# tdavchev/DESIRE

Measured on AMD Instinct MI355X. Metric: agent-trajectory-samples/sec (K=20, T_pred=40), higher is better.
Workload: dtype f32; 1 GPU; BASELINE configs[1]: SDD-like synthetic windows, 32 agent slots/window, K=20, T_obs=8/T_pred=40, H=128, L=128, fp32, posterior CVAE, IOC 1 refinement, social grid 4x4, scene grid 64x64x32; 512 windows/step/GPU; windows_per_gpu=512, rows_per_gpu=327680, parallelism=scene-sharded x1

## Files before the change

### desire_amd/csrc/api_forward.hip

```cpp
#include "ctx.h"

#include <cmath>
#include <cstdio>
#include <cstdlib>
#include <cstring>

bool compact_rows(const desire_ctx* h) { return (h->d.flags & DESIRE_FLAG_COMPACT_ROWS) != 0; }
bool compact_ioc(const desire_ctx* h) { return (h->d.flags & DESIRE_FLAG_COMPACT_IOC) && ioc_plan(h).fwd != IocFwd::STEPWISE; }
ClassLayout class_layout(const desire_ctx* h, bool pad, const int* counts) {
    const desire_dims& d = h->d;
    ClassLayout L;
    int cand[6], nc = 0;
    for (int m : {8, 10, 16, 32, 64, 96}) if (m < d.mno && (m != 10 || pad)) cand[nc++] = m;
    for (int i = nc > 3 ? nc - 3 : 0; i < nc; ++i) L.m[L.n++] = cand[i];
    L.m[L.n++] = d.mno;
    for (int i = L.n; i < 4; ++i) L.m[i] = d.mno;
    for (int c = 0; c < L.n; ++c) {
        IocView& v = L.c[c];
        v.cls = c; v.mno = L.m[c]; v.n_scenes = counts ? counts[c] : d.n_scenes;
        v.gpt = (v.mno <= 32 && 32 % v.mno) ? 32 / v.mno : 0; v.ngrp = v.n_scenes * d.K;
        v.R = v.gpt ? (long)((v.ngrp + v.gpt - 1) / v.gpt) * 32 : (long)v.ngrp * v.mno;
        v.agent_off = L.agents; v.row_off = L.rows; v.win_off = L.wins;
        L.agents += (size_t)v.n_scenes * v.mno; L.rows += (size_t)v.R; L.wins += (size_t)v.n_scenes;
    }
// ... 302 lines not shown

int ioc_cluster_exchange(desire_ctx* h, size_t n_groups, bool reset_err, hipStream_t s) {
    if (!h->ws.count("hex") && (h->ws["hex"].alloc((size_t)2 * h->R * h->d.H * sizeof(float)) || h->ws["grp_cnt"].alloc(((size_t)h->R / 32 + 1) * sizeof(int)) ||
                                h->ws["ioc_err"].alloc(sizeof(int))))
        return fail(DESIRE_ERR_HIP, "hipMalloc failed for the cluster exchange buffers");
    HIPCHK(hipMemsetAsync(h->ws["grp_cnt"].p, 0, n_groups * sizeof(int), s));
    if (reset_err) HIPCHK(hipMemsetAsync(h->ws["ioc_err"].p, 0, sizeof(int), s));
    return DESIRE_OK;
}
int ioc_cluster_check(desire_ctx* h, hipStream_t s, const char* what) {
    int err = 0;
    HIPCHK(hipMemcpyAsync(&err, h->ws["ioc_err"].p, sizeof(int), hipMemcpyDeviceToHost, s));
    HIPCHK(hipStreamSynchronize(s));
    return err ? fail(DESIRE_ERR_HIP, std::string(what) + " hand-off timed out (workgroups of a group were not co-resident)") : DESIRE_OK;
}
#ifdef DESIRE_IOC_TIMING
void ioc_timing_report(const long long* dbg, const char* const* names, int n, hipStream_t s) {
    long long host[16];
    (void)hipStreamSynchronize(s); (void)hipMemcpy(host, dbg, n * sizeof(long long), hipMemcpyDeviceToHost);
    long long tot = 0; for (int k = 0; k < n; ++k) tot += host[k];
    for (int k = 0; k < n; ++k) fprintf(stderr, "[ioc timing] %-45s %12lld cyc  %5.1f%%\n", names[k], host[k], 100.0 * host[k] / (double)tot);
}
#endif

static int ioc_core(desire_handle* h, const IocView& v, hipStream_t s) {
    const desire_dims& d = h->d;
    if (h->training && d.bf16 == 1) return fail(DESIRE_ERR_STATE, "bf16 operands are inference-only");
    IocArgs a{};
    a.Y = v.Y; a.score = v.score; a.Hx = v.Hx; a.ldhx = 2 * d.H; a.p_last = v.p_last; a.valid = v.valid;
    a.R = (int)v.R; a.K = d.K; a.mno = v.mno; a.H = d.H; a.T = d.T_pred; a.iters = d.iters;
    a.C = d.C; a.Gh = d.Gh; a.Gw = d.Gw; a.E_v = d.E_v; a.G = d.grid_size; a.nb_w = d.nb_w; a.nb_h = d.nb_h;
    a.grids = h->grids; a.grid_of_scene = v.gos; a.bin_tab = d.bin_mode == 1 ? W(h, "bin_tab") : nullptr;
    a.w_vel = D(h, "ioc/vel_w"); a.b_vel = D(h, "ioc/vel_b");
    a.Wsoc = D4(h, "ioc/Wsoc"); a.b_soc = D(h, "ioc/soc_b"); a.Wsoc_c = D4(h, "ioc/Wsoc_c");
    a.Wg = D4(h, "ioc/Wg"); a.Wc = D4(h, "ioc/Wc"); a.b_g = D(h, "ioc/gb"); a.b_c = D(h, "ioc/cb");
    a.w_score = D(h, "ioc/score_w"); a.b_score = D(h, "ioc/score_b");
    a.Wreg = D4(h, "ioc/Wreg"); a.b_reg = D(h, "ioc/reg_b"); a.NTreg = (2 * d.T_pred + 31) / 32;
    a.variant = d.ioc_form; a.gpt = v.gpt; a.ngrp = v.ngrp; a.dyn = DynCount{v.dynN, 1, 0};
    const IocPlan p = ioc_plan(d, h->training, v.mno, v.gpt, v.R, [&](int n) { return ioc_bin_split_capacity(a, n); });
    if (!p.fp32_weights()) { a.Wsoc = D4(h, "ioc/Wsoc16"); a.Wg = D4(h, "ioc/Wg16"); a.Wc = D4(h, "ioc/Wc16"); a.Wreg = D4(h, "ioc/Wreg16"); }
    if (p.cluster()) {
        if (int rc = ioc_cluster_exchange(h, (size_t)v.R / v.mno, true, s)) return rc;
        a.hex = W(h, "hex"); a.grp_cnt = static_cast<int*>(h->ws["grp_cnt"].p); a.err = static_cast<int*>(h->ws["ioc_err"].p);
    }
    if (p.nspl > 1) {
        const size_t tiles = ((size_t)v.R + 31) / 32, tiles_max = ((size_t)h->R + 31) / 32;
        if ((!h->ws.count("hex_s") || !h->ws["hex_s"].p || !h->ws["cnt_s"].p) &&
            (h->ws["hex_s"].alloc(tiles_max * 2 * 4 * 32 * d.H * sizeof(float)) || h->ws["cnt_s"].alloc(tiles_max * sizeof(int))))
            return fail(DESIRE_ERR_HIP, "hipMalloc failed for the bin-split exchange buffers");
        if (!h->host_err) {
            if (hipHostMalloc(reinterpret_cast<void**>(&h->host_err), sizeof(int), hipHostMallocMapped) != hipSuccess || !h->host_err)
                { h->host_err = nullptr; return fail(DESIRE_ERR_HIP, "hipHostMalloc failed for the bin-split error word"); }
            *h->host_err = 0;
        }
        if (*static_cast<volatile int*>(h->host_err)) {
            *h->host_err = 0;
            return fail(DESIRE_ERR_HIP, "bin-split IOC hand-off timed out in an earlier call (workgroups of a tile were not co-resident)");
        }
        launch_fill_f32(W(h, "cnt_s"), tiles, 0.f, s);
        a.hex = W(h, "hex_s"); a.grp_cnt = static_cast<int*>(h->ws["cnt_s"].p); a.err = h->host_err;
        a.nspl = p.nspl;
    }
#ifdef DESIRE_IOC_TIMING
    if (!h->ws.count("dbg")) { h->ws["dbg"].alloc(10 * sizeof(long long)); }
    a.dbg = static_cast<long long*>(h->ws["dbg"].p);
#endif
    const int passes = h->training ? d.iters : 1;
// ... 130 lines not shown
```

### desire_amd/csrc/api_pack.hip

```cpp
#include "ctx.h"

#include <cmath>
#include <cstdio>
#include <cstdlib>
#include <cstring>

namespace {
void fold_bn(desire_ctx* h, const std::string& p, std::vector<float>& scale, std::vector<float>& shift) {
    const auto& g = h->host_w.at(p + "/bn/gamma"); const auto& be = h->host_w.at(p + "/bn/beta");
    const auto& mu = h->host_w.at(p + "/bn/moving_mean"); const auto& var = h->host_w.at(p + "/bn/moving_var");
    const auto& b = h->host_w.at(p + "/b");
    scale.resize(g.size()); shift.resize(g.size());
    for (size_t i = 0; i < g.size(); ++i) {
        const double sc = (double)g[i] / std::sqrt((double)var[i] + 1e-3);
        scale[i] = (float)sc;
        shift[i] = (float)((double)be[i] + sc * ((double)b[i] - (double)mu[i]));
    }
}

}

int desire_pack_all(desire_ctx* h) {
    const desire_dims& d = h->d;
    const int H = d.H, L = d.L, V = h->V, E = h->E, B = h->B;
// ... 200 lines not shown
                return out;
            };
            bad |= up("vae_enc/conv2/W16", fwd16(hw["vae_enc/conv2/w"], 32, 64));
            bad |= up("vae_enc/conv3/W16", fwd16(hw["vae_enc/conv3/w"], 64, 128));
        }
        bad |= up("vae_dec/deconv2/W16", taps16(hw["vae_dec/deconv2/w"], 128, 64));
        bad |= up("vae_dec/deconv3/W16", taps16(hw["vae_dec/deconv3/w"], 64, 32));
        {
            const auto& w4 = hw["vae_dec/deconv4/w"];
            bad |= up("vae_dec/deconv4/W16", pack_b16(32, 32, chain, [&](int k, int n) { return n < 25 ? w4[(size_t)n * 32 + k] : 0.f; }));
        }
    }
    bad |= up("ioc/vel_w", hw["ioc/vel_fc/w"]); bad |= up("ioc/vel_b", hw["ioc/vel_fc/b"]);
    {
        std::vector<float> all;
        for (int b = 0; b < B; ++b) {
            auto pk = pack_b(H, H, rowmajor(hw["ioc/social_fc/w"], H, b * H));
            all.insert(all.end(), pk.begin(), pk.end());
        }
        bad |= up("ioc/Wsoc", all);
    }
    {
        const auto& ws = hw["ioc/social_fc/w"];
        const int T16 = H / 16;
        std::vector<float> all((size_t)B * H * H);
        for (int b = 0; b < B; ++b)
            for (int ct = 0; ct < T16; ++ct)
                for (int g = 0; g < T16; ++g)
                    for (int lane = 0; lane < 64; ++lane)
                        for (int j = 0; j < 4; ++j)
                            all[((((size_t)b * T16 + ct) * T16 + g) * 64 + lane) * 4 + j] =
                                ws[((size_t)b * H + 16 * g + 4 * (lane >> 4) + j) * H + 16 * ct + (lane & 15)];
        bad |= up("ioc/Wsoc_c", all);
    }
    bad |= up("ioc/soc_b", hw["ioc/social_fc/b"]);
    bad |= up("ioc/score_w", hw["ioc/score/w"]); bad |= up("ioc/score_b", hw["ioc/score/b"]);
    bad |= up("ioc/Wreg", pack_b(H, 2 * d.T_pred, rowmajor(hw["ioc/reg/w"], 2 * d.T_pred, 0)));
    bad |= up("ioc/reg_b", hw["ioc/reg/b"]);
    bad |= up("fc_c/W", pack_b(2 * H, V, rowmajor(hw["fc_c/w"], V, 0)));  bad |= up("fc_c/b", hw["fc_c/b"]);
    bad |= up("vae_enc/fc/W", pack_b(2048, 2 * L, rowmajor(hw["vae_enc/fc/w"], 2 * L, 0)));
    bad |= up("vae_enc/fc/b", hw["vae_enc/fc/b"]);
    bad |= up("mask/W", pack_b(V, H, rowmajor(hw["mask_fc/w"], H, 0)));  bad |= up("mask/b", hw["mask_fc/b"]);
    std::vector<float> sc, sh;
    for (const char* n : {"vae_enc/conv1", "vae_enc/conv2", "vae_enc/conv3", "vae_dec/deconv1", "vae_dec/deconv2",
                          "vae_dec/deconv3", "vae_dec/deconv4"}) {
        fold_bn(h, n, sc, sh);
        bad |= up(std::string(n) + "/scale", sc); bad |= up(std::string(n) + "/shift", sh);
        if (d.bn_mode != 0) { bad |= up(std::string(n) + "/gamma", hw[std::string(n) + "/bn/gamma"]); bad |= up(std::string(n) + "/beta", hw[std::string(n) + "/bn/beta"]); }
    }
    bad |= up("vae_enc/conv1/raw", hw["vae_enc/conv1/w"]);
    bad |= up("vae_dec/deconv4/raw", hw["vae_dec/deconv4/w"]);
    auto pack_taps = [&](const std::vector<float>& w, int CI, int CO, bool transposed) {
        std::vector<float> all;
        for (int tap = 0; tap < 25; ++tap) {
            const float* base = w.data() + (size_t)tap * CI * CO;
            auto pk = pack_b(CI, CO, [&](int k, int n) { return transposed ? base[(size_t)n * CI + k] : base[(size_t)k * CO + n]; });
            all.insert(all.end(), pk.begin(), pk.end());
        }
        return all;
    };
    bad |= up("vae_enc/conv2/W", pack_taps(hw["vae_enc/conv2/w"], 32, 64, false));
    bad |= up("vae_enc/conv3/W", pack_taps(hw["vae_enc/conv3/w"], 64, 128, false));
    bad |= up("vae_dec/deconv2/W", pack_taps(hw["vae_dec/deconv2/w"], 128, 64, true));
    bad |= up("vae_dec/deconv3/W", pack_taps(hw["vae_dec/deconv3/w"], 64, 32, true));
    {
        const auto& w1 = hw["vae_dec/deconv1/w"];
// ... 22 lines not shown
```

### desire_amd/csrc/kernels.h

```cpp
#pragma once
#include <hip/hip_runtime.h>
#include <stdint.h>

template <class F>
inline void allow_big_lds(F* f) {
    static bool done = false;
    if (!done) {
        (void)hipFuncSetAttribute(reinterpret_cast<const void*>(f), hipFuncAttributeMaxDynamicSharedMemorySize, 160 * 1024);
        done = true;
    }
}

struct DynCount { const int32_t* cnt; int mul; int hint; };
inline int dyn_units(int worst, const DynCount& d) {
    if (!d.cnt || d.hint <= 0) return worst;
    const long g = (long)d.hint * d.mul, want = g + g / 4 + 256;
    return (int)(want < (long)worst ? want : (long)worst);
}

enum { EPI_BIAS = 0, EPI_BIAS_RELU = 1, EPI_SCALE_SHIFT_ELU = 2, EPI_NONE = 3, EPI_ELUGRAD = 4, EPI_SIGGRAD = 5 };

struct GemmArgs {
    const float* A; int lda; int M; int K;
    const float4* Bp; int G; int NT;
// ... 47 lines not shown
    uint8_t* valid;
    float* sv_r; float* sv_u; float* sv_c; float* sv_h; float* sv_x;
    int n_roll; const float* w5; const float* b5;
    const float* normals; float* roll_out;
    DynCount dyn;
};
void launch_encoder(const EncArgs& a, hipStream_t s);
void launch_encoder_pair(const EncArgs& past, const EncArgs& fut, hipStream_t s);
void launch_encoder_bf16(const EncArgs& a, hipStream_t s);

struct DecArgs {
    const float* xz; const float* Hx; int ldhx; const float* p_last;
    int R; int K; int mno; int H; int T;
    const float4* Wxg; const float4* Wxc; const float4* Whg; const float4* Whc;
    const float* b_g; const float* b_c;
    const float* w_head; const float* b_head;
    float* Y;
    float* hdump;
    float* sv_r; float* sv_u; float* sv_c;
    DynCount dyn;
};
void launch_decoder(const DecArgs& a, hipStream_t s);
void launch_decoder_bf16(const DecArgs& a, hipStream_t s);

struct IocArgs {
    float* Y; float* score;
    const float* Hx; int ldhx; const float* p_last; const uint8_t* valid;
    int R; int K; int mno; int H; int T; int iters;
    int C; int Gh; int Gw; int E_v; int G; float nb_w, nb_h;
    const float* grids; const int32_t* grid_of_scene;
    const float* w_vel; const float* b_vel;
    const float4* Wsoc; const float* b_soc;
    const float4* Wsoc_c;
    const float4* Wg; const float4* Wc; const float* b_g; const float* b_c;
    const float* w_score; const float* b_score;
    const float4* Wreg; const float* b_reg; int NTreg;
    int variant;
    long long* dbg;
    float* hex; int* grp_cnt; int* err;
    int nspl;
    float* sv_x; float* sv_r; float* sv_u; float* sv_c; float* sv_h;
    const float* bin_tab;
    int gpt; int ngrp;
    DynCount dyn;
};
void launch_ioc(const IocArgs& a, bool wide, hipStream_t s);
void launch_ioc_cluster(const IocArgs& a, hipStream_t s);
int ioc_bin_split_capacity(const IocArgs& a, int n);
void launch_ioc_bf16(const IocArgs& a, bool wide, hipStream_t s);
int launch_ioc_bf16_cluster(const IocArgs& a, hipStream_t s);
void launch_ioc_x3(const IocArgs& a, hipStream_t s);
void launch_ioc_x6(const IocArgs& a, hipStream_t s);
void launch_ioc_x6r2(const IocArgs& a, hipStream_t s);
void launch_ioc_x3r2(const IocArgs& a, hipStream_t s);
bool decoder_x6_supported(int H);
void launch_decoder_x6(const DecArgs& a, hipStream_t s, int np = 3);
void launch_deconv2_x6(const ConvArgs& a, hipStream_t s, int np = 3);
void launch_deconv3_x6(const ConvArgs& a, hipStream_t s, int np = 3);
struct IocStepArgs {
    int t; int rank; int nranks; int m_loc; int n_scenes; int K; int R;
    int H; int T; int Gh; int Gw; int G; float nb_w, nb_h;
    const float* Yall; const float* plast_all; const uint8_t* valid_all; const float* Hall;
    int peer; const float* Yp[8]; const float* plp[8]; const uint8_t* vp[8]; const float* Hp[8];
    const float* st_h; float* st_h_out; float* st_score; float* st_h_copy;
    const float* grids; const int32_t* grid_of_scene;
    const float* w_vel; const float* b_vel; const float4* Wsoc; const float* b_soc;
// ... 138 lines not shown
```

### desire_amd/csrc/kernels_rnn.hip

```cpp
#include "common.h"
#include "kernels.h"
#include <cstdlib>
#include <map>
#include <tuple>

#define RNN_WG 512

__device__ __forceinline__ f32x16 splat16(float v) {
    f32x16 z;
#pragma unroll
    for (int i = 0; i < 16; ++i) z[i] = v;
    return z;
}

__device__ __forceinline__ void mma1(f32x16& acc, const float* a_lane, const float4* __restrict__ b_lane, int G) {
    f32x16 t[1] = {acc};
    mma_groups<1>(t, a_lane, 0, b_lane, G);
    acc = t[0];
}

template <int H, int TM, bool ROLL>
__device__ __forceinline__ void encoder_tile(const EncArgs& a, int blk) {
    extern __shared__ __attribute__((aligned(16))) float smem[];
    constexpr int LDH = H + 4, NT = H >> 5, G = H >> 3, NTHR = NT * (TM / 32) * 64;
// ... 289 lines not shown
    }
}
template <int H, int TM>
static void launch_decoder_t(const DecArgs& a, hipStream_t s) {
    const size_t lds = (2 * TM * (H + 4) + 2 * H + TM * 2) * sizeof(float);
    if (a.sv_r || a.sv_c || a.hdump) {
        allow_big_lds(k_decoder<H, TM, true>);
        hipLaunchKernelGGL((k_decoder<H, TM, true>), dim3((a.R + TM - 1) / TM), dim3((H / 32) * (TM / 32) * 64), lds, s, a);
    } else {
        allow_big_lds(k_decoder<H, TM, false>);
        hipLaunchKernelGGL((k_decoder<H, TM, false>), dim3((a.R + TM - 1) / TM), dim3((H / 32) * (TM / 32) * 64), lds, s, a);
    }
}
void launch_decoder(const DecArgs& a, hipStream_t s) {
    if (a.H == 256) launch_decoder_t<256, 32>(a, s);
    else if (a.H == 128) {
        launch_decoder_t<128, 32>(a, s);
    }
    else launch_decoder_t<64, 64>(a, s);
}

#include "cluster.h"
#include "split.h"
template <int TM> struct MaskT { typedef unsigned long long type; };
template <> struct MaskT<32> { typedef unsigned type; };
__device__ __forceinline__ int ffs_(unsigned m) { return __ffs((int)m); }
__device__ __forceinline__ int ffs_(unsigned long long m) { return __ffsll((long long)m); }
#ifdef DESIRE_IOC_TIMING
#define TICK(k) { const long long now_ = clock64(); tacc[k] += now_ - tprev; tprev = now_; }
#else
#define TICK(k)
#endif
typedef float f32x4v __attribute__((ext_vector_type(4)));
template <int H, int EV, int C, int TM, bool TRAIN, bool CP = false, int NSPL = 1, bool PAD = false>
__global__ __launch_bounds__((H / 32) * (TM / 32) * 64, ((H / 32) * (TM / 32) <= 2) ? 1 : 2) void k_ioc(IocArgs a) {
#ifdef DESIRE_IOC_TIMING
    long long tacc[10] = {0, 0, 0, 0, 0, 0, 0, 0, 0, 0};
    long long tprev = clock64();
#endif
    extern __shared__ __attribute__((aligned(16))) float smem[];
    constexpr int NT = H >> 5, E = EV + C + H, KX = E + H, LDX = KX + 4, LDB = H + 4;
    constexpr int NTHR = NT * (TM / 32) * 64, TPR = NTHR / TM;
    constexpr int G8 = KX >> 3, GH = H >> 3;
    constexpr int NCH = H / (4 * TPR);
    const int B = a.G * a.G;
    float* XH = smem;
    float* AB = XH + (TM + 1) * LDX;
    typedef typename MaskT<TM>::type mask_t;
    mask_t* masks = reinterpret_cast<mask_t*>(AB + 2 * TM * LDB);
    float* pc = reinterpret_cast<float*>(masks + TM * B);
    float* pp = pc + TM * 2;
    float* wv = pp + TM * 2;
    float* red = wv + 3 * EV;
    unsigned char* vld = reinterpret_cast<unsigned char*>(red + NT * TM);
    unsigned* occ = reinterpret_cast<unsigned*>(vld + TM);
    unsigned* rowbits = occ + 2;
    unsigned* rowlist = rowbits + 36;

    const int lane = lane_id(), w = wave_id(), tid = threadIdx.x;
    const int cb = w % NT, mt = w / NT;
    const int tile = NSPL > 1 ? (int)blockIdx.x / NSPL : (int)blockIdx.x, member = NSPL > 1 ? (int)blockIdx.x % NSPL : 0;
    const int row0 = tile * TM;
    IOC_DYN(a)
    if (a.dyn.cnt && row0 >= a.R) return;
    unsigned long long my_bins = ~0ull;
    if (NSPL > 1) { my_bins = 0ull; for (int b = member; b < 64; b += NSPL) my_bins |= 1ull << b; }
    const bool active = cb < NT;
    const int col = cb * 32 + (lane & 31);
// ... 23 lines not shown
    constexpr int NS = 2;
    auto build = [&](int b, int buf) {
        float* ab = AB + buf * TM * LDB + r8 * LDB;
        mask_t m2 = masks[r8 * B + b];
        int off[NS];
#pragma unroll
        for (int sl = 0; sl < NS; ++sl) {
            off[sl] = m2 ? (grp_base + ffs_(m2) - 1) * LDX : TM * LDX;
            m2 &= m2 - 1;
        }
        float4 s[NCH];
#pragma unroll
        for (int c = 0; c < NCH; ++c) {
            const float4 v0 = *reinterpret_cast<const float4*>(XH + off[0] + E + q8 * 4 + c * 4 * TPR);
            const float4 v1 = *reinterpret_cast<const float4*>(XH + off[1] + E + q8 * 4 + c * 4 * TPR);
            s[c].x = v0.x + v1.x; s[c].y = v0.y + v1.y; s[c].z = v0.z + v1.z; s[c].w = v0.w + v1.w;
        }
        if (__any(m2 != 0)) {
            while (m2) {
                const int j = ffs_(m2) - 1;
                m2 &= m2 - 1;
                const float* src = XH + (grp_base + j) * LDX + E + q8 * 4;
#pragma unroll
                for (int c = 0; c < NCH; ++c) {
                    const float4 v = *reinterpret_cast<const float4*>(src + c * 4 * TPR);
                    s[c].x += v.x; s[c].y += v.y; s[c].z += v.z; s[c].w += v.w;
                }
            }
        }
#pragma unroll
        for (int c = 0; c < NCH; ++c) *reinterpret_cast<float4*>(ab + q8 * 4 + c * 4 * TPR) = s[c];
    };

    for (int it = 0; it < a.iters; ++it) {
        for (int i = tid; i < TM * (H >> 2); i += NTHR) {
            const int r = i / (H >> 2), c4 = i - r * (H >> 2);
            const int ag = ioc_agent_of_row(min(row0 + r, a.R - 1), a.K, a.mno, gpt, a.ngrp);
            *reinterpret_cast<float4*>(XH + r * LDX + E + c4 * 4) =
                ag >= 0 ? *reinterpret_cast<const float4*>(a.Hx + (size_t)ag * a.ldhx + c4 * 4) : make_float4(0.f, 0.f, 0.f, 0.f);
        }
        if (tid < TM) {
            const int ag = ioc_agent_of_row(min(row0 + tid, a.R - 1), a.K, a.mno, gpt, a.ngrp);
            pp[tid * 2] = ag >= 0 ? a.p_last[(size_t)ag * 2] : 0.f;
            pp[tid * 2 + 1] = ag >= 0 ? a.p_last[(size_t)ag * 2 + 1] : 0.f;
        }
        __syncthreads();
        f32x16 h = zero16(), sp = zero16();
        if (active) {
#pragma unroll
            for (int i = 0; i < 16; ++i) h[i] = my_x[((i & 3) + 8 * (i >> 2)) * LDX + E];
        }

        float2 ynext = make_float2(0.f, 0.f);
        if (tid < TM) {
            const float2 y0 = *reinterpret_cast<const float2*>(a.Y + ((size_t)min(row0 + tid, a.R - 1) * a.T) * 2);
            pc[tid * 2] = y0.x; pc[tid * 2 + 1] = y0.y;
        }
        for (int i = tid; i < TM * B; i += NTHR) masks[i] = 0;
        if (tid < 2) occ[tid] = 0;
        if (CP && tid < B) rowbits[tid] = 0;
        __syncthreads();
        const float* rh_lane = AB + (mt * 32 + (lane & 31)) * LDB + 4 * (lane >> 5);
        float* my_rh = AB + (mt * 32 + 4 * (lane >> 5)) * LDB + col;
        constexpr int GX = E >> 3;

        for (int t = 0; t < a.T; ++t) {
            TICK(0)
            if (tid < TM && t + 1 < a.T)
                ynext = *reinterpret_cast<const float2*>(a.Y + ((size_t)min(row0 + tid, a.R - 1) * a.T + t + 1) * 2);
            {
                const float px = pc[r8 * 2], py = pc[r8 * 2 + 1];
                const float vx = px - pp[r8 * 2], vy = py - pp[r8 * 2 + 1];
                constexpr int per = EV / TPR;
#pragma unroll
                for (int j = q8 * per; j < (q8 + 1) * per; ++j)
                    XH[r8 * LDX + j] = fmaxf(fmaf(vy, wv[EV + j], vx * wv[j]) + wv[2 * EV + j], 0.f);
                int cy, cx;
                scene_cell_dev(px, py, a.Gh, a.Gw, cy, cx);
                const float* gsrc = grid + ((size_t)cy * a.Gw + cx) * C;
                constexpr int cper = C / TPR;
                if (cper >= 4) {
#pragma unroll
                    for (int j = q8 * cper; j < (q8 + 1) * cper; j += 4)
                        *reinterpret_cast<float4*>(XH + r8 * LDX + EV + j) = *reinterpret_cast<const float4*>(gsrc + j);
                } else {
                    *reinterpret_cast<float2*>(XH + r8 * LDX + EV + q8 * 2) = *reinterpret_cast<const float2*>(gsrc + q8 * 2);
                }
                float nbw, nbh;
                nb_opaque(a.nb_w, a.nb_h, nbw, nbh);
                const unsigned long long oc = nb_search<4>(pc, vld, grp_base, n_nb, q8, TPR, my_slot, px, py, nbw, nbh, a.G, a.bin_tab,
                                                          [&](int j, int b) {
                                                              atomicOr(&masks[r8 * B + b], (mask_t)1 << j);
                                                              if (CP) atomicOr(&rowbits[b], 1u << r8);
                                                          });
                nb_publish_occ(oc, occ, B);
                if (CP) {
#pragma unroll
                    for (int c = 0; c < NCH; ++c)
                        *reinterpret_cast<float4*>(XH + r8 * LDX + EV + C + q8 * 4 + c * 4 * TPR) = make_float4(0.f, 0.f, 0.f, 0.f);
                }
            }
            __syncthreads();
            TICK(1)
            if constexpr (CP) {
                unsigned long long om = (unsigned long long)__builtin_amdgcn_readfirstlane((int)occ[0]) & 0xffffffffull;
                om |= (unsigned long long)(unsigned)__builtin_amdgcn_readfirstlane((int)occ[1]) << 32;
                constexpr int T16 = H / 16;
                auto build_c = [&](int b, int buf) {
                    const unsigned rb = rowbits[b];
                    if (!((rb >> r8) & 1u)) return;
                    const int slot = __popc(rb & ((1u << r8) - 1u));
                    float* ab = AB + buf * TM * LDB + slot * LDB;
                    mask_t m2 = masks[r8 * B + b];
                    const int o0 = (grp_base + ffs_(m2) - 1) * LDX;
                    m2 &= m2 - 1;
                    const int o1 = m2 ? (grp_base + ffs_(m2) - 1) * LDX : TM * LDX;
                    m2 &= m2 - 1;
                    float4 sacc[NCH];
#pragma unroll
                    for (int c = 0; c < NCH; ++c) {
                        const float4 v0 = *reinterpret_cast<const float4*>(XH + o0 + E + q8 * 4 + c * 4 * TPR);
                        const float4 v1 = *reinterpret_cast<const float4*>(XH + o1 + E + q8 * 4 + c * 4 * TPR);
                        sacc[c].x = v0.x + v1.x; sacc[c].y = v0.y + v1.y; sacc[c].z = v0.z + v1.z; sacc[c].w = v0.w + v1.w;
                    }
                    while (m2) {
                        const int j = ffs_(m2) - 1;
                        m2 &= m2 - 1;
                        const float* src = XH + (grp_base + j) * LDX + E + q8 * 4;
#pragma unroll
                        for (int c = 0; c < NCH; ++c) {
                            const float4 v = *reinterpret_cast<const float4*>(src + c * 4 * TPR);
                            sacc[c].x += v.x; sacc[c].y += v.y; sacc[c].z += v.z; sacc[c].w += v.w;
                        }
                    }
#pragma unroll
                    for (int c = 0; c < NCH; ++c) *reinterpret_cast<float4*>(ab + q8 * 4 + c * 4 * TPR) = sacc[c];
                    if (q8 == 0) reinterpret_cast<unsigned char*>(rowlist + buf * (TM / 4))[slot] = (unsigned char)r8;
                };
                int buf = 0;
                if (om) build_c(ffs_(om) - 1, 0);
                __syncthreads();
                while (om) {
                    const int b = ffs_(om) - 1;
                    om &= om - 1;
                    const float4* w0 = a.Wsoc_c + ((size_t)(b * T16 + 2 * cb) * T16) * 64 + lane;
                    float4 wf[2][T16];
                    if (active) {
#pragma unroll
                        for (int g = 0; g < T16; ++g) { wf[0][g] = w0[g * 64]; wf[1][g] = w0[(T16 + g) * 64]; }
                    }
                    if (om) build_c(ffs_(om) - 1, buf ^ 1);
                    const int nrows = __popc(__builtin_amdgcn_readfirstlane((int)rowbits[b]));
                    if (active) {
                        for (int c16 = 0; c16 * 16 < nrows; ++c16) {
                            f32x4v a0 = {0.f, 0.f, 0.f, 0.f}, a1 = {0.f, 0.f, 0.f, 0.f};
                            const float* ap = AB + buf * TM * LDB + (16 * c16 + (lane & 15)) * LDB + 4 * (lane >> 4);
#pragma unroll
                            for (int g = 0; g < T16; ++g) {
                                const float4 av = *reinterpret_cast<const float4*>(ap + 16 * g);
                                a0 = __builtin_amdgcn_mfma_f32_16x16x4f32(av.x, wf[0][g].x, a0, 0, 0, 0);
                                a1 = __builtin_amdgcn_mfma_f32_16x16x4f32(av.x, wf[1][g].x, a1, 0, 0, 0);
                                a0 = __builtin_amdgcn_mfma_f32_16x16x4f32(av.y, wf[0][g].y, a0, 0, 0, 0);
                                a1 = __builtin_amdgcn_mfma_f32_16x16x4f32(av.y, wf[1][g].y, a1, 0, 0, 0);
                                a0 = __builtin_amdgcn_mfma_f32_16x16x4f32(av.z, wf[0][g].z, a0, 0, 0, 0);
                                a1 = __builtin_amdgcn_mfma_f32_16x16x4f32(av.z, wf[1][g].z, a1, 0, 0, 0);
                                a0 = __builtin_amdgcn_mfma_f32_16x16x4f32(av.w, wf[0][g].w, a0, 0, 0, 0);
                                a1 = __builtin_amdgcn_mfma_f32_16x16x4f32(av.w, wf[1][g].w, a1, 0, 0, 0);
                            }
                            const unsigned rl4 = rowlist[buf * (TM / 4) + 4 * c16 + (lane >> 4)];
                            float* ex = XH + EV + C + cb * 32 + (lane & 15);
#pragma unroll
// ... 101 lines not shown
                }
#pragma unroll
                for (int i = 0; i < 16; ++i) my_rh[((i & 3) + 8 * (i >> 2)) * LDB] = rh[i];
#pragma unroll
                for (int i = 0; i < 16; ++i) {
                    u[i] = sigmoidf_(u[i] + bgu);
                    if (TRAIN && row0 + mt * 32 + acc_row(i) < a.R) sv_u_t[sv_off(i, t)] = u[i];
                }
            }
            __syncthreads();
            TICK(7)
            if (active) {
                f32x16 ac = zero16();
                mma1(ac, x_lane, a.Wc + ((size_t)cb * G8) * 64 + lane, GX);
                mma1(ac, rh_lane, a.Wc + ((size_t)cb * G8 + GX) * 64 + lane, GH);
#pragma unroll
                for (int i = 0; i < 16; ++i) {
                    const float c = tanhf_(ac[i] + bcc);
                    h[i] = gru_blend(u[i], h[i], c);
                    sp[i] = fmaf(h[i], wsc, sp[i]);
                    if (TRAIN && row0 + mt * 32 + acc_row(i) < a.R) { sv_c_t[sv_off(i, t)] = c; sv_h_t[sv_off(i, t)] = h[i]; }
                }
#pragma unroll
                for (int i = 0; i < 16; ++i)
                    my_x[((i & 3) + 8 * (i >> 2)) * LDX + E] = h[i];
            }
            __builtin_amdgcn_s_setprio(0);
            if (tid < TM) {
                pp[tid * 2] = pc[tid * 2]; pp[tid * 2 + 1] = pc[tid * 2 + 1];
                pc[tid * 2] = ynext.x; pc[tid * 2 + 1] = ynext.y;
            }
            for (int i = tid; i < TM * B; i += NTHR) masks[i] = 0;
            if (tid < 2) occ[tid] = 0;
            if (CP && tid < B) rowbits[tid] = 0;
            __syncthreads();
            TICK(8)
        }
#pragma unroll
        for (int i = 0; i < 16; ++i) {
            float v = active ? sp[i] : 0.f;
            v += __shfl_xor(v, 1); v += __shfl_xor(v, 2); v += __shfl_xor(v, 4);
            v += __shfl_xor(v, 8); v += __shfl_xor(v, 16);
            if ((lane & 31) == 0) red[cb * TM + mt * 32 + acc_row(i)] = v;
        }
        __syncthreads();
        bool poisoned = false;
        if constexpr (NSPL > 1) poisoned = __hip_atomic_load(a.err, __ATOMIC_RELAXED, __HIP_MEMORY_SCOPE_SYSTEM) != 0;
        if (tid < TM && row0 + tid < a.R && it == a.iters - 1 && member == 0) {
            float sc = 0.f;
#pragma unroll
            for (int c = 0; c < NT; ++c) sc += red[c * TM + tid];
            a.score[row0 + tid] = poisoned ? __builtin_nanf("") : sc + (float)a.T * a.b_score[0];
        }
        for (int nt = cb; nt < a.NTreg; nt += NT) {
            f32x16 acc = zero16();
            mma1(acc, x_lane + E, a.Wreg + ((size_t)nt * GH) * 64 + lane, GH);
            const int cc = nt * 32 + (lane & 31);
            if (cc < 2 * a.T) {
                const float bb = a.b_reg[cc];
#pragma unroll
                for (int i = 0; i < 16; ++i) {
                    const int row = row0 + mt * 32 + acc_row(i);
                    if (row < a.R && member == 0) {
                        float* y = a.Y + (size_t)row * 2 * a.T + cc;
                        *y = poisoned ? __builtin_nanf("") : *y + (acc[i] + bb);
                    }
                }
// ... 26 lines not shown
            if (a.variant != 9) {
                allow_big_lds(k_ioc<H, 16, 32, 32, true, true>);
                hipLaunchKernelGGL((k_ioc<H, 16, 32, 32, true, true>), grid, block, ioc_lds_bytes(a, TM), s, a);
                return;
            }
        }
        if constexpr (H <= 128 || TM == 32) {
            allow_big_lds(k_ioc<H, 16, 32, TM, true>);
            hipLaunchKernelGGL((k_ioc<H, 16, 32, TM, true>), grid, block, ioc_lds_bytes(a, TM), s, a);
        }
        return;
    }
    if constexpr (TM == 32 && H <= 128) {
        if (a.variant == 8) {
            allow_big_lds(k_ioc<H, 16, 32, 32, false, true>);
            hipLaunchKernelGGL((k_ioc<H, 16, 32, 32, false, true>), grid, block, ioc_lds_bytes(a, TM), s, a);
            return;
        }
    }
    if constexpr (TM == 32 && H <= 128) {
        if (a.nspl > 1) {
            const dim3 gs(grid.x * a.nspl);
            switch (a.nspl) {
                case 3: allow_big_lds(k_ioc<H, 16, 32, 32, false, false, 3>); hipLaunchKernelGGL((k_ioc<H, 16, 32, 32, false, false, 3>), gs, block, ioc_lds_bytes(a, TM), s, a); return;
                case 4: allow_big_lds(k_ioc<H, 16, 32, 32, false, false, 4>); hipLaunchKernelGGL((k_ioc<H, 16, 32, 32, false, false, 4>), gs, block, ioc_lds_bytes(a, TM), s, a); return;
                default: allow_big_lds(k_ioc<H, 16, 32, 32, false, false, 2>); hipLaunchKernelGGL((k_ioc<H, 16, 32, 32, false, false, 2>), gs, block, ioc_lds_bytes(a, TM), s, a); return;
            }
        }
    }
    if constexpr (TM == 32 && H <= 128) {
        if (a.gpt > 0) {
            allow_big_lds(k_ioc<H, 16, 32, 32, false, false, 1, true>);
            hipLaunchKernelGGL((k_ioc<H, 16, 32, 32, false, false, 1, true>), grid, block, ioc_lds_bytes(a, TM), s, a);
            return;
        }
    }
    allow_big_lds(k_ioc<H, 16, 32, TM, false>);
    hipLaunchKernelGGL((k_ioc<H, 16, 32, TM, false>), grid, block, ioc_lds_bytes(a, TM), s, a);
}
int ioc_bin_split_capacity(const IocArgs& a, int n) {
    if (a.mno > 32 || a.H > 128 || n < 2 || n > 4) return 0;
    static std::map<std::tuple<int, int, int, size_t>, int> cache;
    int dev = 0;
    if (hipGetDevice(&dev) != hipSuccess) return 0;
    const size_t lds = ioc_lds_bytes(a, 32);
    const auto key = std::make_tuple(dev, a.H, n, lds);
    auto it = cache.find(key);
    if (it != cache.end()) return it->second;
    const void* kern = nullptr;
    if (a.H == 128) kern = n == 2 ? (const void*)k_ioc<128, 16, 32, 32, false, false, 2> : n == 3 ? (const void*)k_ioc<128, 16, 32, 32, false, false, 3> : (const void*)k_ioc<128, 16, 32, 32, false, false, 4>;
    else kern = n == 2 ? (const void*)k_ioc<64, 16, 32, 32, false, false, 2> : n == 3 ? (const void*)k_ioc<64, 16, 32, 32, false, false, 3> : (const void*)k_ioc<64, 16, 32, 32, false, false, 4>;
    (void)hipFuncSetAttribute(kern, hipFuncAttributeMaxDynamicSharedMemorySize, 160 * 1024);
    int per_cu = 0, cus = 0;
    int cap = 0;
    if (hipOccupancyMaxActiveBlocksPerMultiprocessor(&per_cu, kern, (a.H / 32) * 64, lds) == hipSuccess && per_cu > 0 &&
        hipDeviceGetAttribute(&cus, hipDeviceAttributeMultiprocessorCount, dev) == hipSuccess)
        cap = per_cu * cus;
    cache[key] = cap;
    return cap;
}
void launch_ioc(const IocArgs& a, bool wide, hipStream_t s) {
    if (a.H == 256) launch_ioc_t<256, 32>(a, s);
    else if (a.H == 128) { if (wide) launch_ioc_t<128, 64>(a, s); else launch_ioc_t<128, 32>(a, s); }
    else { if (wide) launch_ioc_t<64, 64>(a, s); else launch_ioc_t<64, 32>(a, s); }
}

// ... 854 lines not shown
```

Before: 2.417 million samples/s.

## Add row-sparse social pooling path to IOC kernel using compacted per-bin row lists

Adds an SP template variant of the IOC kernel that pools only the rows that actually have neighbours in each occupied bin. Those rows are gathered into compacted 16-row MFMA tiles, instead of running the full 32-row tile for every occupied bin. A new Wsoc_s weight layout with a permuted k ordering is packed to match this gather scheme. The build_c lambda is hoisted so it can be shared with the existing compact path. The new path is dispatched for non-padded inference when the variant is not 9. The aim is to cut wasted MFMA work on sparse neighbour bins, at the cost of extra gather/scatter LDS traffic and added synchronisation per bin.

```diff
diff --git a/desire_amd/csrc/api_forward.hip b/desire_amd/csrc/api_forward.hip
--- a/desire_amd/csrc/api_forward.hip
+++ b/desire_amd/csrc/api_forward.hip
@@ -358,7 +358,7 @@
     a.C = d.C; a.Gh = d.Gh; a.Gw = d.Gw; a.E_v = d.E_v; a.G = d.grid_size; a.nb_w = d.nb_w; a.nb_h = d.nb_h;
     a.grids = h->grids; a.grid_of_scene = v.gos; a.bin_tab = d.bin_mode == 1 ? W(h, "bin_tab") : nullptr;
     a.w_vel = D(h, "ioc/vel_w"); a.b_vel = D(h, "ioc/vel_b");
-    a.Wsoc = D4(h, "ioc/Wsoc"); a.b_soc = D(h, "ioc/soc_b"); a.Wsoc_c = D4(h, "ioc/Wsoc_c");
+    a.Wsoc = D4(h, "ioc/Wsoc"); a.b_soc = D(h, "ioc/soc_b"); a.Wsoc_c = D4(h, "ioc/Wsoc_c"); a.Wsoc_s = D4(h, "ioc/Wsoc_s");
     a.Wg = D4(h, "ioc/Wg"); a.Wc = D4(h, "ioc/Wc"); a.b_g = D(h, "ioc/gb"); a.b_c = D(h, "ioc/cb");
     a.w_score = D(h, "ioc/score_w"); a.b_score = D(h, "ioc/score_b");
     a.Wreg = D4(h, "ioc/Wreg"); a.b_reg = D(h, "ioc/reg_b"); a.NTreg = (2 * d.T_pred + 31) / 32;
diff --git a/desire_amd/csrc/api_pack.hip b/desire_amd/csrc/api_pack.hip
--- a/desire_amd/csrc/api_pack.hip
+++ b/desire_amd/csrc/api_pack.hip
@@ -256,6 +256,15 @@
                             all[((((size_t)b * T16 + ct) * T16 + g) * 64 + lane) * 4 + j] =
                                 ws[((size_t)b * H + 16 * g + 4 * (lane >> 4) + j) * H + 16 * ct + (lane & 15)];
         bad |= up("ioc/Wsoc_c", all);
+        for (int b = 0; b < B; ++b)
+            for (int ct = 0; ct < T16; ++ct)
+                for (int g = 0; g < T16; ++g)
+                    for (int lane = 0; lane < 64; ++lane)
+                        for (int j = 0; j < 4; ++j) {
+                            const int q = lane >> 4, k = 16 * g + 8 * (j >> 1) + 2 * (j & 1) + 4 * (q & 1) + (q >> 1);
+                            all[((((size_t)b * T16 + ct) * T16 + g) * 64 + lane) * 4 + j] = ws[((size_t)b * H + k) * H + 16 * ct + (lane & 15)];
+                        }
+        bad |= up("ioc/Wsoc_s", all);
     }
     bad |= up("ioc/soc_b", hw["ioc/social_fc/b"]);
     bad |= up("ioc/score_w", hw["ioc/score/w"]); bad |= up("ioc/score_b", hw["ioc/score/b"]);
diff --git a/desire_amd/csrc/kernels.h b/desire_amd/csrc/kernels.h
--- a/desire_amd/csrc/kernels.h
+++ b/desire_amd/csrc/kernels.h
@@ -103,6 +103,7 @@
     const float* w_vel; const float* b_vel;
     const float4* Wsoc; const float* b_soc;
     const float4* Wsoc_c;
+    const float4* Wsoc_s;
     const float4* Wg; const float4* Wc; const float* b_g; const float* b_c;
     const float* w_score; const float* b_score;
     const float4* Wreg; const float* b_reg; int NTreg;
diff --git a/desire_amd/csrc/kernels_rnn.hip b/desire_amd/csrc/kernels_rnn.hip
--- a/desire_amd/csrc/kernels_rnn.hip
+++ b/desire_amd/csrc/kernels_rnn.hip
@@ -345,8 +345,10 @@
 #define TICK(k)
 #endif
 typedef float f32x4v __attribute__((ext_vector_type(4)));
-template <int H, int EV, int C, int TM, bool TRAIN, bool CP = false, int NSPL = 1, bool PAD = false>
+template <int H, int EV, int C, int TM, bool TRAIN, bool CP = false, int NSPL = 1, bool PAD = false, bool SP = false>
 __global__ __launch_bounds__((H / 32) * (TM / 32) * 64, ((H / 32) * (TM / 32) <= 2) ? 1 : 2) void k_ioc(IocArgs a) {
+    static_assert(!SP || (TM == 32 && !TRAIN && !CP && NSPL == 1), "row-sparse pooling: 32-row inference tiles of the plain form only");
+    constexpr bool RC = CP || SP;
 #ifdef DESIRE_IOC_TIMING
     long long tacc[10] = {0, 0, 0, 0, 0, 0, 0, 0, 0, 0};
     long long tprev = clock64();
@@ -436,6 +438,38 @@
         for (int c = 0; c < NCH; ++c) *reinterpret_cast<float4*>(ab + q8 * 4 + c * 4 * TPR) = s[c];
     };
 
+    auto build_c = [&](int b, int buf) {
+        const unsigned rb = rowbits[b];
+        if (!((rb >> r8) & 1u)) return;
+        const int slot = __popc(rb & ((1u << r8) - 1u));
+        float* ab = AB + buf * TM * LDB + slot * LDB;
+        mask_t m2 = masks[r8 * B + b];
+        const int o0 = (grp_base + ffs_(m2) - 1) * LDX;
+        m2 &= m2 - 1;
+        const int o1 = m2 ? (grp_base + ffs_(m2) - 1) * LDX : TM * LDX;
+        m2 &= m2 - 1;
+        float4 sacc[NCH];
+#pragma unroll
+        for (int c = 0; c < NCH; ++c) {
+            const float4 v0 = *reinterpret_cast<const float4*>(XH + o0 + E + q8 * 4 + c * 4 * TPR);
+            const float4 v1 = *reinterpret_cast<const float4*>(XH + o1 + E + q8 * 4 + c * 4 * TPR);
+            sacc[c].x = v0.x + v1.x; sacc[c].y = v0.y + v1.y; sacc[c].z = v0.z + v1.z; sacc[c].w = v0.w + v1.w;
+        }
+        while (m2) {
+            const int j = ffs_(m2) - 1;
+            m2 &= m2 - 1;
+            const float* src = XH + (grp_base + j) * LDX + E + q8 * 4;
+#pragma unroll
+            for (int c = 0; c < NCH; ++c) {
+                const float4 v = *reinterpret_cast<const float4*>(src + c * 4 * TPR);
+                sacc[c].x += v.x; sacc[c].y += v.y; sacc[c].z += v.z; sacc[c].w += v.w;
+            }
+        }
+#pragma unroll
+        for (int c = 0; c < NCH; ++c) *reinterpret_cast<float4*>(ab + q8 * 4 + c * 4 * TPR) = sacc[c];
+        if (q8 == 0) reinterpret_cast<unsigned char*>(rowlist + buf * (TM / 4))[slot] = (unsigned char)r8;
+    };
+
     for (int it = 0; it < a.iters; ++it) {
         for (int i = tid; i < TM * (H >> 2); i += NTHR) {
             const int r = i / (H >> 2), c4 = i - r * (H >> 2);
@@ -462,7 +496,7 @@
         }
         for (int i = tid; i < TM * B; i += NTHR) masks[i] = 0;
         if (tid < 2) occ[tid] = 0;
-        if (CP && tid < B) rowbits[tid] = 0;
+        if (RC && tid < B) rowbits[tid] = 0;
         __syncthreads();
         const float* rh_lane = AB + (mt * 32 + (lane & 31)) * LDB + 4 * (lane >> 5);
         float* my_rh = AB + (mt * 32 + 4 * (lane >> 5)) * LDB + col;
@@ -495,10 +529,10 @@
                 const unsigned long long oc = nb_search<4>(pc, vld, grp_base, n_nb, q8, TPR, my_slot, px, py, nbw, nbh, a.G, a.bin_tab,
                                                           [&](int j, int b) {
                                                               atomicOr(&masks[r8 * B + b], (mask_t)1 << j);
-                                                              if (CP) atomicOr(&rowbits[b], 1u << r8);
+                                                              if (RC) atomicOr(&rowbits[b], 1u << r8);
                                                           });
                 nb_publish_occ(oc, occ, B);
-                if (CP) {
+                if (RC) {
 #pragma unroll
                     for (int c = 0; c < NCH; ++c)
                         *reinterpret_cast<float4*>(XH + r8 * LDX + EV + C + q8 * 4 + c * 4 * TPR) = make_float4(0.f, 0.f, 0.f, 0.f);
@@ -506,41 +540,77 @@
             }
             __syncthreads();
             TICK(1)
-            if constexpr (CP) {
+            if constexpr (SP) {
                 unsigned long long om = (unsigned long long)__builtin_amdgcn_readfirstlane((int)occ[0]) & 0xffffffffull;
                 om |= (unsigned long long)(unsigned)__builtin_amdgcn_readfirstlane((int)occ[1]) << 32;
                 constexpr int T16 = H / 16;
-                auto build_c = [&](int b, int buf) {
-                    const unsigned rb = rowbits[b];
-                    if (!((rb >> r8) & 1u)) return;
-                    const int slot = __popc(rb & ((1u << r8) - 1u));
-                    float* ab = AB + buf * TM * LDB + slot * LDB;
-                    mask_t m2 = masks[r8 * B + b];
-                    const int o0 = (grp_base + ffs_(m2) - 1) * LDX;
-                    m2 &= m2 - 1;
-                    const int o1 = m2 ? (grp_base + ffs_(m2) - 1) * LDX : TM * LDX;
-                    m2 &= m2 - 1;
-                    float4 sacc[NCH];
-#pragma unroll
-                    for (int c = 0; c < NCH; ++c) {
-                        const float4 v0 = *reinterpret_cast<const float4*>(XH + o0 + E + q8 * 4 + c * 4 * TPR);
-                        const float4 v1 = *reinterpret_cast<const float4*>(XH + o1 + E + q8 * 4 + c * 4 * TPR);
-                        sacc[c].x = v0.x + v1.x; sacc[c].y = v0.y + v1.y; sacc[c].z = v0.z + v1.z; sacc[c].w = v0.w + v1.w;
-                    }
-                    while (m2) {
-                        const int j = ffs_(m2) - 1;
-                        m2 &= m2 - 1;
-                        const float* src = XH + (grp_base + j) * LDX + E + q8 * 4;
-#pragma unroll
-                        for (int c = 0; c < NCH; ++c) {
-                            const float4 v = *reinterpret_cast<const float4*>(src + c * 4 * TPR);
-                            sacc[c].x += v.x; sacc[c].y += v.y; sacc[c].z += v.z; sacc[c].w += v.w;
+                int buf = 0;
+                if (om) build_c(ffs_(om) - 1, 0);
+                __syncthreads();
+                __builtin_amdgcn_s_setprio(3);
+                const int q = lane >> 4;
+                float* ex = XH + EV + C + cb * 32 + (lane & 15);
+                const int kq = 4 * (q & 1) + (q >> 1);
+                float4 wf[2][T16];
+                auto load_w = [&](int b) {
+                    const float4* w0 = a.Wsoc_s + ((size_t)(b * T16 + 2 * cb) * T16) * 64 + lane;
+#pragma unroll
+                    for (int g = 0; g < T16; ++g) { wf[0][g] = w0[g * 64]; wf[1][g] = w0[(T16 + g) * 64]; }
+                };
+                int ro[4];
+                f32x4v a0, a1;
+                auto gather = [&](int c16, int nrows) {
+                    const unsigned rl4 = rowlist[buf * (TM / 4) + 4 * c16 + q];
+#pragma unroll
+                    for (int i = 0; i < 4; ++i) {
+                        ro[i] = 16 * c16 + 4 * q + i < nrows ? (int)((rl4 >> (8 * i)) & 0xffu) * LDX : -1;
+                        a0[i] = ro[i] >= 0 ? ex[ro[i]] : 0.f;
+                        a1[i] = ro[i] >= 0 ? ex[ro[i] + 16] : 0.f;
+                    }
+                };
+                while (om) {
+                    const int b = ffs_(om) - 1;
+                    om &= om - 1;
+                    if (active) load_w(b);
+                    const int nrows = __popc(__builtin_amdgcn_readfirstlane((int)rowbits[b]));
+                    if (om) build_c(ffs_(om) - 1, buf ^ 1);
+                    if (active) {
+                        for (int c16 = 0; c16 * 16 < nrows; ++c16) {
+                            gather(c16, nrows);
+                            const float* ap = AB + buf * TM * LDB + (16 * c16 + (lane & 15)) * LDB + kq;
+#pragma unroll
+                            for (int g = 0; g < T16; ++g) {
+                                const float x0 = ap[16 * g], x1 = ap[16 * g + 2], x2 = ap[16 * g + 8], x3 = ap[16 * g + 10];
+                                a0 = __builtin_amdgcn_mfma_f32_16x16x4f32(x0, wf[0][g].x, a0, 0, 0, 0);
+                                a1 = __builtin_amdgcn_mfma_f32_16x16x4f32(x0, wf[1][g].x, a1, 0, 0, 0);
+                                a0 = __builtin_amdgcn_mfma_f32_16x16x4f32(x1, wf[0][g].y, a0, 0, 0, 0);
+                                a1 = __builtin_amdgcn_mfma_f32_16x16x4f32(x1, wf[1][g].y, a1, 0, 0, 0);
+                                a0 = __builtin_amdgcn_mfma_f32_16x16x4f32(x2, wf[0][g].z, a0, 0, 0, 0);
+                                a1 = __builtin_amdgcn_mfma_f32_16x16x4f32(x2, wf[1][g].z, a1, 0, 0, 0);
+                                a0 = __builtin_amdgcn_mfma_f32_16x16x4f32(x3, wf[0][g].w, a0, 0, 0, 0);
+                                a1 = __builtin_amdgcn_mfma_f32_16x16x4f32(x3, wf[1][g].w, a1, 0, 0, 0);
+                            }
+#pragma unroll
+                            for (int i = 0; i < 4; ++i) {
+                                if (ro[i] >= 0) { ex[ro[i]] = a0[i]; ex[ro[i] + 16] = a1[i]; }
+                            }
                         }
                     }
-#pragma unroll
-                    for (int c = 0; c < NCH; ++c) *reinterpret_cast<float4*>(ab + q8 * 4 + c * 4 * TPR) = sacc[c];
-                    if (q8 == 0) reinterpret_cast<unsigned char*>(rowlist + buf * (TM / 4))[slot] = (unsigned char)r8;
-                };
+                    __syncthreads();
+                    buf ^= 1;
+                }
+                __builtin_amdgcn_s_setprio(0);
+                if (active) {
+#pragma unroll
+                    for (int i = 0; i < 16; ++i) {
+                        float* e = my_x + ((i & 3) + 8 * (i >> 2)) * LDX + EV + C;
+                        *e = fmaxf(*e + bso, 0.f);
+                    }
+                }
+            } else if constexpr (CP) {
+                unsigned long long om = (unsigned long long)__builtin_amdgcn_readfirstlane((int)occ[0]) & 0xffffffffull;
+                om |= (unsigned long long)(unsigned)__builtin_amdgcn_readfirstlane((int)occ[1]) << 32;
+                constexpr int T16 = H / 16;
                 int buf = 0;
                 if (om) build_c(ffs_(om) - 1, 0);
                 __syncthreads();
@@ -708,7 +778,7 @@
             }
             for (int i = tid; i < TM * B; i += NTHR) masks[i] = 0;
             if (tid < 2) occ[tid] = 0;
-            if (CP && tid < B) rowbits[tid] = 0;
+            if (RC && tid < B) rowbits[tid] = 0;
             __syncthreads();
             TICK(8)
         }
@@ -801,6 +871,11 @@
         if (a.gpt > 0) {
             allow_big_lds(k_ioc<H, 16, 32, 32, false, false, 1, true>);
             hipLaunchKernelGGL((k_ioc<H, 16, 32, 32, false, false, 1, true>), grid, block, ioc_lds_bytes(a, TM), s, a);
+            return;
+        }
+        if (a.variant != 9) {
+            allow_big_lds(k_ioc<H, 16, 32, 32, false, false, 1, false, true>);
+            hipLaunchKernelGGL((k_ioc<H, 16, 32, 32, false, false, 1, false, true>), grid, block, ioc_lds_bytes(a, TM), s, a);
             return;
         }
     }
diff --git a/profiles/ab/sparse_fill.py b/profiles/ab/sparse_fill.py
--- /dev/null
+++ b/profiles/ab/sparse_fill.py
@@ -0,0 +1,54 @@
+import argparse
+import os
+import sys
+
+import numpy as np
+
+sys.path.insert(0, os.path.dirname(os.path.dirname(os.path.dirname(os.path.abspath(__file__)))))
+from desire_amd.spec import Dims, init_weights
+from desire_amd.synth import make_case
+from oracle import desire_oracle as O
+
+
+def main():
+    ap = argparse.ArgumentParser()
+    ap.add_argument("--windows", type=int, default=8)
+    ap.add_argument("--nb", type=float, default=0.15)
+    ap.add_argument("--grid", type=int, default=4)
+    ap.add_argument("--seed", type=int, default=0)
+    a = ap.parse_args()
+    d = Dims(n_scenes=a.windows, mno=32, K=20, T_obs=8, T_pred=40, H=128, L=128, n_grids=1, grid_size=a.grid, nb_w=a.nb, nb_h=a.nb,
+             sx=1.0 / 1400.0, sy=1.0 / 1100.0, iters=1, posterior=1)
+    w = init_weights(d, a.seed)
+    past, fut, eps, grids, gos = make_case(d, seed=a.seed + 1, n_absent=0)
+    tr = lambda x: np.ascontiguousarray(x.transpose(1, 0, 2, 3).reshape(x.shape[1], -1, 3))
+    Y0 = O.forward(tr(past), tr(fut), eps, grids, gos, w, d)["Y0"]
+    B = d.grid_size ** 2
+    valid = np.ones((d.n_scenes * d.K, d.mno), bool)
+    hist = np.zeros(d.mno + 1, np.int64)
+    occupied = dense_rows = sparse_rows = 0
+    for t in range(d.T_pred):
+        P = Y0[:, t].reshape(d.n_scenes * d.K, d.mno, 2)
+        bins = O.neighbor_bins(P, valid, d.nb_w, d.nb_h, d.grid_size)
+        has = (bins[..., None] == np.arange(B)).any(axis=2)
+        n = has.sum(axis=1)
+        hist += np.bincount(n.ravel(), minlength=d.mno + 1)
+        occ = n > 0
+        occupied += int(occ.sum())
+        sparse_rows += int((np.ceil(n / 16) * 16).sum())
+    tiles_steps = d.n_scenes * d.K * d.T_pred
+    dense_rows = occupied * 32
+    print("windows %d, tiles x steps %d, bins %d, nb %.3f" % (d.n_scenes, tiles_steps, B, d.nb_w))
+    print("rows with a neighbour per (tile, step, bin): histogram (rows: share of all (tile, step, bin))")
+    for k in range(d.mno + 1):
+        if hist[k]:
+            print("  %2d: %.4f" % (k, hist[k] / hist.sum()))
+    nz = hist[1:] * np.arange(1, d.mno + 1)
+    print("occupied bins per (tile, step): %.2f of %d; mean rows per occupied bin %.2f; bins with > 16 rows: %.4f of occupied" % (
+        occupied / tiles_steps, B, nz.sum() / hist[1:].sum(), hist[17:].sum() / hist[1:].sum()))
+    print("pooling MFMA rows executed: dense kernel %d (occupied bins x 32), row-sparse %d (16-row tiles) = %.3f of the dense kernel, %.3f of the "
+          "dense formula (all bins x 32)" % (dense_rows, sparse_rows, sparse_rows / dense_rows, sparse_rows / (tiles_steps * B * 32)))
+
+
+if __name__ == "__main__":
+    main()
```

New measurement: 2.722 million samples/s, median of 6. 12.6% higher.
